# zrudnick/bramble

Hardware: AMD Instinct MI355X
Metric: projected alignments/sec vs GENCODE-scale annotation (higher is better)
Workload: dtype u32; 1 GPU; device-resident (inputs already in HBM, packed rows left in HBM): 10M paired-end 2x100 short reads (name-collated, unstranded) vs GENCODE-shaped synthetic annotation (250836 transcripts, 1684128 transcript-exon rows, 25 refs); BASELINE.json configs[1]; group_lanes=8, seed=0xb4a3b1e

## Files before the change

bramble_amd/csrc/abi.cpp:

```cpp
#include <hip/hip_runtime.h>

#include <algorithm>
#include <atomic>
#include <cstdio>
#include <cstdlib>
#include <cstring>
#include <functional>
#include <string>
#include <thread>
#include <unordered_map>
#include <vector>

#include "ctx.h"
#include "primary_pick.h"

int check_device(int device) {
  int n = 0;
  hipError_t e = hipGetDeviceCount(&n);
  if (e != hipSuccess || n <= 0 || device >= n) return BR_ERR_NO_DEVICE;
  return BR_OK;
}

template <typename T>
static int upload(void **dst, const std::vector<T> &src, size_t &acc) {
// ... 342 lines not shown
  return BR_OK;
}

extern "C" void br_ctx_free(br_ctx *c) {
  if (!c) return;
  (void)hipSetDevice(c->ix->device);
  for (auto &e : c->events) { (void)hipEventDestroy(e.a); (void)hipEventDestroy(e.b); }
  if (c->rb) (void)hipHostFree(c->rb);
  for (auto &S : c->stage) if (S.ready) (void)hipEventDestroy(S.ready);
  for (auto &S : c->in_slot) {
    if (S.ready) (void)hipEventDestroy(S.ready);
    if (S.rows_home) (void)hipEventDestroy(S.rows_home);
  }
  if (c->rows_busy) (void)hipEventDestroy(c->rows_busy);
  if (c->alt.busy) (void)hipEventDestroy(c->alt.busy);
  if (c->side2_stream) (void)hipStreamDestroy(c->side2_stream);
  if (c->side_stream) { (void)hipStreamDestroy(c->side_stream); for (auto &p : c->side_ev) for (auto &e : p) if (e) (void)hipEventDestroy(e); }
  if (c->run_stream) (void)hipStreamDestroy(c->run_stream);
  if (c->d2h_stream) (void)hipStreamDestroy(c->d2h_stream);
  if (c->copy_stream) (void)hipStreamDestroy(c->copy_stream);
  if (c->down_stream) (void)hipStreamDestroy(c->down_stream);
  for (int k = 0; k < 2; k++) if (c->ev_home[k]) (void)hipEventDestroy(c->ev_home[k]);
  delete c;
}

extern "C" int br_ctx_set_profiling(br_ctx *c, int enabled) {
  if (!c) return BR_ERR_INVALID_ARG;
  if (enabled && !c->profiling) for (int k = 0; k < BR_K_NUM; k++) { c->k_ms_sum[k] = 0; c->k_launches_sum[k] = 0; }
  c->profiling = enabled != 0;
  return BR_OK;
}
extern "C" int br_ctx_kernel_ms_sum(br_ctx *c, int which, double *ms, int64_t *launches) {
  if (!c || which < 0 || which >= BR_K_NUM) return BR_ERR_INVALID_ARG;
  if (ms) *ms = c->k_ms_sum[which];
  if (launches) *launches = c->k_launches_sum[which];
  return BR_OK;
}
extern "C" int br_ctx_set_param(br_ctx *c, const char *key, int64_t v) {
  if (!c || !key) return BR_ERR_INVALID_ARG;
  if (!strcmp(key, "group_lanes")) { if (v != 8 && v != 16 && v != 32 && v != 64) return BR_ERR_INVALID_ARG; c->group_lanes = (int)v; return BR_OK; }
  if (!strcmp(key, "direct_rows")) { c->direct_rows = v != 0; return BR_OK; }
  if (!strcmp(key, "small_batch")) { c->small_batch = v != 0; return BR_OK; }
  if (!strcmp(key, "speculate")) { c->speculate = v != 0; return BR_OK; }
  if (!strcmp(key, "speculate_n")) { if (v < 0) return BR_ERR_INVALID_ARG; c->speculate_n = v; return BR_OK; }
  if (!strcmp(key, "small_n")) { if (v < 0) return BR_ERR_INVALID_ARG; c->small_n = v; return BR_OK; }
  if (!strcmp(key, "deflate_dynamic")) { c->deflate_dynamic = v != 0; return BR_OK; }
  if (!strcmp(key, "bam_lanes")) { if (v != 0 && v != 4 && v != 8 && v != 16 && v != 32 && v != 64) return BR_ERR_INVALID_ARG; c->bam_lanes = (int)v; return BR_OK; }
  if (!strcmp(key, "ksw_fast")) { c->ksw_fast = v != 0; return BR_OK; }
  if (!strcmp(key, "ksw_tape_pct")) { if (v < 0 || v > 100) return BR_ERR_INVALID_ARG; c->ksw_tape_pct = (int)v; return BR_OK; }
  if (!strcmp(key, "ksw_tape_mb")) { if (v < 1) return BR_ERR_INVALID_ARG; c->ksw_tape_mb = v; return BR_OK; }
  if (!strcmp(key, "host_detail")) { c->host_detail = v != 0; return BR_OK; }
  if (!strcmp(key, "split_spoil")) { if (v < 0 || v > 1000000) return BR_ERR_INVALID_ARG; c->split_spoil = (int)v; return BR_OK; }
  if (!strcmp(key, "side_cap")) { if (v < 64) return BR_ERR_INVALID_ARG; c->d_side_cap = (uint64_t)v; return BR_OK; }
  if (!strcmp(key, "blocks_per_cu")) { if (v < 1 || v > 64) return BR_ERR_INVALID_ARG; c->blocks_per_cu = (int)v; return BR_OK; }
  return BR_ERR_INVALID_ARG;
}
extern "C" int br_ctx_kernel_ms(br_ctx *c, int which, double *ms, int32_t *launches) {
  if (!c || which < 0 || which >= BR_K_NUM) return BR_ERR_INVALID_ARG;
  if (ms) *ms = c->k_ms[which];
  if (launches) *launches = c->k_launches[which];
  return BR_OK;
}
extern "C" int br_ctx_ksw_diag(br_ctx *c, uint64_t out[16]) {
  if (!c || !out) return BR_ERR_INVALID_ARG;
  memcpy(out, c->ksw_diag, sizeof(c->ksw_diag));
  out[7] = (uint32_t)c->rb->ksw_left_after;
  return BR_OK;
}

extern "C" int br_ctx_rescue_stats(br_ctx *c, uint64_t out[4]) {
  if (!c || !out) return BR_ERR_INVALID_ARG;
  memcpy(out, c->rescue_stats, sizeof(c->rescue_stats));
  return BR_OK;
}
extern "C" int br_ctx_last_counters(br_ctx *c, uint64_t out[8]) {
  if (!c || !out) return BR_ERR_INVALID_ARG;
  memcpy(out, c->counters, sizeof(c->counters));
  return BR_OK;
}

extern "C" int br_pin_host(void *p, size_t bytes) {
  if (!p || !bytes) return BR_ERR_INVALID_ARG;
  HIPCHK(hipHostRegister(p, bytes, hipHostRegisterDefault));
  return BR_OK;
}
extern "C" int br_unpin_host(void *p) {
  if (!p) return BR_ERR_INVALID_ARG;
  HIPCHK(hipHostUnregister(p));
  return BR_OK;
}

extern "C" uint32_t br_primary_pick(const char *name, size_t len, uint32_t n_tied) {
  return n_tied ? br::primary_pick((const uint8_t *)name, len, n_tied) : 0;
}

extern "C" uint32_t br_row_mapq(uint32_t nh, int long_reads) {
  if (!long_reads) return nh == 1 ? 255u : nh == 2 ? 3u : (nh == 3 || nh == 4) ? 1u : 0u;
  return nh > 1 ? 0u : 3u;
}

extern "C" int br_device_warmup(int device) {
  int rc = check_device(device);
  if (rc) return rc;
  HIPCHK(hipSetDevice(device));
  HIPCHK(hipFree(nullptr));
  return BR_OK;
// ... 16 lines not shown
```

bramble_amd/csrc/ctx.h:

```cpp
#pragma once
#include <hip/hip_runtime.h>

#include <atomic>
#include <cassert>
#include <string>
#include <vector>

#include "../../include/bramble_amd.h"
#include "device_types.h"
#include "devmem.h"
#include "kernels.h"

using namespace br;

struct br_index {
  int device = -1;
  std::vector<std::string> names;
  std::vector<uint32_t> lengths;
  uint32_t n_refs = 0;
  bool has_seq = false;
  std::vector<uint32_t> slab_off, s_start, s_pmax, s_tid, tx_first, bin_off;
  std::vector<uint4> t_bin;
  std::vector<uint4> s_row, tx_ex;
  std::vector<uint8_t> seq_pool;
  void *d_slab_off = nullptr, *d_s_start = nullptr, *d_s_pmax = nullptr, *d_bin_off = nullptr, *d_t_bin = nullptr, *d_s_tid = nullptr,
       *d_s_row = nullptr, *d_tx_ex = nullptr, *d_tx_first = nullptr, *d_seq_pool = nullptr;
  size_t device_bytes = 0;
  DevIndex dev{};
};

struct KEvent { int which; hipEvent_t a, b; };

struct ReadBack {
  uint64_t scan[5];
  uint64_t counters[4];
  uint64_t small[TOT_SMALL_CNT + 4];
  uint64_t direct_cnt[GD_COUNTER_WORDS];
  uint64_t side[2];
  uint64_t wide_cigar;
  uint64_t rescue_n[2];
  uint64_t rescue_stats[2];
  uint32_t ksw_bins[16];
  uint64_t ksw_left_after;
  uint64_t parse_n[3];
  uint64_t parse_seq;
  uint64_t parse_max;
  uint64_t bam[2];
  uint64_t deflate_total;
  uint64_t host_groups, host_max, host_pool;
  uint64_t sam_bad, sam_bytes;
};

struct br_ctx {
  const br_index *ix = nullptr;
  int group_lanes = 8;
  int bam_lanes = 0;
  int blocks_per_cu = 8;
  int split_spoil = 0;
  int n_cu = 256;
  bool profiling = false;
  std::vector<KEvent> events; size_t events_used = 0;
  double k_ms[BR_K_NUM] = {0}; int32_t k_launches[BR_K_NUM] = {0};
  double k_ms_sum[BR_K_NUM] = {0}; int64_t k_launches_sum[BR_K_NUM] = {0};
  uint64_t counters[8] = {0};
  uint64_t rescue_stats[4] = {0};
  DevBuf seg, meta, head, head2, fast_flag, fast_pre, n_matches, ranges, mask, match_off, cig_base, tile_sums, totals, counters_d;
  DevBuf m_tid, m_aux, m_p, m_x, m_b, m_cigoff, cig_arena, big_list, n_big, m_aln;
  DevBuf bam_aux, bam_base, bam_len, bam_off, bam_out, bam_end;
  struct StageSlot { DevBuf blob, off, len; hipEvent_t ready = nullptr; std::vector<uint64_t> h_off; int64_t n = 0; };
  StageSlot stage[3];
  hipStream_t copy_stream = nullptr;
  struct InSlot {
    DevBuf ref_id, ref_start, flags, xs, ts, cigar_off64, cigar, mate_ref, mate_start, name_off64, names, lqseq, seq_off64, seqs;
    DevBuf cigar_off, name_off, seq_off, mate_idx, group_off, seq_src, isnew, group_pre;
    hipEvent_t ready = nullptr, rows_home = nullptr;
    int64_t n = -1; uint64_t n_words = 0, n_name = 0, n_seq = 0; bool has_seq = false, staged = false, rows_pending = false;
    PinnedVec<uint4> h_a; PinnedVec<uint64_t> h_c, h_row_off; PinnedVec<uint32_t> h_pool; PinnedVec<uint4> h_x;
    PinnedVec<int32_t> h_mate, h_clip; PinnedVec<double> h_sim;
  };
  InSlot in_slot[2];
  hipStream_t run_stream = nullptr, d2h_stream = nullptr;
  hipEvent_t rows_busy = nullptr;
  bool rows_busy_set = false;
  struct RowSetAlt { DevBuf pk_a, pk_x, pk_sim, pk_clip, pk_ch, pool, row_off; hipEvent_t busy = nullptr; bool busy_set = false; } alt;
  int host_detail = 0;
  DevBuf z_slots, z_sizes, z_off, z_dense, z_dense_alt, z_tabs, z_tokens;
  DevBuf inf_out, inf_blocks, inf_tabs, inf_cnt; bool inf_tabs_ready = false;
  DevBuf sp_entry, sp_entry2, sp_exit, sp_nmap, sp_nunm, sp_ended, sp_redo, sp_pre, sp_small, sp_off, sp_len;
  DevBuf sf_names, sf_name_off, sf_len, sf_long, sf_small, sf_tmp, sf_text[2];
  int32_t sf_n_names = 0;
  int sf_which = 0;
  int z_dense_which = 0;
  hipStream_t down_stream = nullptr; hipEvent_t ev_home[2] = {nullptr, nullptr}; std::atomic<bool> home_pending[2] = {{false}, {false}};
  int deflate_dynamic = 1;
  int64_t speculate_n = 4194304;
  int speculate = 1;
  int64_t hist_n = 0; uint64_t hist[4] = {0, 0, 0, 0}; bool hist_simf = false;
  int small_batch = 1;
  int64_t small_n = 65536;
  DevBuf walk_list, pmask, pbit, pick;
  int direct_rows = 1;
  DevBuf d_fm, d_nkept, d_desc, d_hi0, d_clspos, d_rnd, d_side, d_sidectr;
  uint64_t d_side_cap = 0;
  int d_side_attempts = 0;
  bool last_direct = false;
  bool want_x = false;
  ProjectArgs dA{}; DirectArgs dD{}; int64_t d_kept = 0, d_simple = 0;
  DevBuf r_rec, pk_a, pk_c, pk_x, pk_sim, pk_clip;
  DevBuf pool, pool_sizes, pool_off, pk_ch;
  bool last_aux_cols = false;
  bool wide_valid = false;
  bool detail_valid = false;
  const int32_t *last_l_qseq = nullptr;
  int32_t last_long_reads = 0;
  int64_t last_n_pool = 0;
  bool z_tabs_ready = false;
  DevBuf p_ncig, p_name_len, p_isnew, p_group_pre, p_small, p_big, p_seq_len, p_ref_map;
  uint8_t *h_bam[2] = {nullptr, nullptr}; size_t h_bam_cap[2] = {0, 0}; int h_bam_next = 0;
  BigPinned h_bam_mem[2];
  int64_t last_n_rows = 0, last_n_aln = 0;
  br_device_bam last_bam{};
  br_device_rows last_rows{}; const uint32_t *last_group_off = nullptr; int64_t last_n_groups = 0; hipStream_t last_stream = nullptr;
  DevBuf fa_stats, fa_n_prob, fa_seq_bytes, fa_prob_off, fa_seqarena_off, fa_probs, fa_results, fa_seq_arena, fa_clip_ops,
      fa_ideal_cap, fa_scratch, fa_srcs, fa_want, b_seq_off, b_seqs, b_seq_src;
  DevBuf ksw_desc, ksw_dp, ksw_left, ksw_cnt, ksw_group, ksw_tape, ksw_raw;
  int ksw_fast = 1;
  hipStream_t side_stream = nullptr, side2_stream = nullptr;
  static constexpr int SIDE_EV = 8;
  hipEvent_t side_ev[SIDE_EV][2] = {}; int side_live = 0;
  uint32_t ksw_groups[KSW_N_BINS] = {0};
  int64_t ksw_tape_mb = 49152;
  int ksw_tape_pct = 100;
  uint64_t ksw_diag[16] = {0};
  DevBuf n_rows, row_off, aln_group;
  DevBuf r_input, r_nh, r_hi, r_mapq, r_group, r_mate_tid, r_mate_pos,
      r_isize, r_tid, r_pos, r_ncig, r_strand, r_sim, r_clip, r_junc, r_refc, r_cigoff, cigar_out;
  DevBuf r_paired, r_same, r_first, r_primary;
  DevBuf b_name_off, b_names;
  DevBuf b_ref_id, b_ref_start, b_flags, b_xs, b_ts, b_cigar_off, b_cigar, b_mate_idx, b_group_off, b_lqseq;
  ReadBack *rb = nullptr;
  PinnedVec<int32_t> h_input, h_clip, h_junc, h_refc, h_mate_tid, h_mate_pos, h_isize;
  PinnedVec<uint32_t> h_tid, h_pos, h_nh, h_hi, h_mapq, h_group, h_cigar;
  PinnedVec<int8_t> h_strand;
  PinnedVec<uint64_t> h_cigoff;
  PinnedVec<double> h_sim;
  PinnedVec<uint8_t> h_primary, h_paired, h_same, h_first;
  std::vector<br_projected> h_proj;
  PinnedVec<uint8_t> g_host; DevBuf g_dev;
  PinnedVec<uint4> g_a, g_x; PinnedVec<uint2> g_c; PinnedVec<uint32_t> g_pool, g_cig; PinnedVec<double> g_sim;
  bool rows_to_host = false, rows_at_host = false;
};

struct Prof {
  br_ctx *c; hipStream_t st;
  hipStream_t cur = nullptr;
  int begin(int which, hipStream_t on = nullptr) {
// ... 70 lines not shown
```

bramble_amd/csrc/direct_kernels.inc:

```

#define WAVE_SYNC()                                                \
  do {                                                             \
    __builtin_amdgcn_fence(__ATOMIC_RELEASE, "workgroup");         \
    __builtin_amdgcn_wave_barrier();                               \
    __builtin_amdgcn_fence(__ATOMIC_ACQUIRE, "workgroup");         \
  } while (0)

__global__ void __launch_bounds__(256) k_name_seed(DirectArgs D) {
  const int64_t g = (int64_t)blockIdx.x * blockDim.x + threadIdx.x;
  if (g >= D.n_groups) return;
  const uint32_t a0 = D.group_off[g];
  const uint32_t no = D.name_off[a0];
  Mt64Lazy gen;
  gen.seed(hash_bytes(D.names + no, D.name_off[a0 + 1] - no));
  D.rnd0[g] = gen();
}
__device__ __forceinline__ uint32_t pick_from(uint64_t z0, const uint8_t *name, uint64_t len, uint32_t n) {
  uint64_t hi, lo;
  mul64wide(z0, (uint64_t)n, hi, lo);
  if (lo < (uint64_t)n) {
    const uint64_t thr = (0 - (uint64_t)n) % (uint64_t)n;
    if (lo < thr) return primary_pick(name, len, n);
  }
  return (uint32_t)hi;
// ... 479 lines not shown
    if (small) {
#pragma unroll
      for (int k = 0; k < 4; k++) {
        const uint32_t i = a0 + (uint32_t)k, r = r4[k];
        if (r) {
        const uint32_t pf = f4[k];
        const bool paired = (pf & PF_PAIRED) != 0;
        const uint32_t u = paired ? r / 2 : r;
        uint32_t prim = 0;
        if (have_prim && idx != 0xffffffffu) { if (idx < u) { prim = idx + 1u; idx = 0xffffffffu; } else idx -= u; }
        D.gd[i] = make_uint2(pf | (prim << 8), total);
        D.hi0[i] = run + 1u;
        if (paired) {
          const uint32_t m = (uint32_t)mi4[k], mk = m - a0;
          const uint32_t pfm = mk < na ? (mk == 0 ? f4[0] : mk == 1 ? f4[1] : mk == 2 ? f4[2] : f4[3]) : (uint32_t)D.pflag[m];
          D.gd[m] = make_uint2(pfm | (prim << 8), total);
          D.hi0[m] = run + 2u;
        }
        run += r;
        }
      }
    } else {
      for (uint32_t i = a0; i < a1; i++) {
        const uint32_t r = D.n_rows[i];
        if (!r) continue;
        const uint32_t pf = D.pflag[i];
        const bool paired = (pf & PF_PAIRED) != 0;
        const uint32_t u = paired ? r / 2 : r;
        uint32_t prim = 0;
        if (have_prim && idx != 0xffffffffu) { if (idx < u) { prim = idx + 1u; idx = 0xffffffffu; } else idx -= u; }
        D.gd[i] = make_uint2(pf | (prim << 8), total);
        D.hi0[i] = run + 1u;
        if (paired) {
          const uint32_t m = (uint32_t)D.mate_idx[i];
          D.gd[m] = make_uint2((uint32_t)D.pflag[m] | (prim << 8), total);
          D.hi0[m] = run + 2u;
        }
        run += r;
      }
    }
  }
  __shared__ unsigned long long sh_c[4][2];
  uniq = wave_sum(uniq); dropped = wave_sum(dropped);
  if ((threadIdx.x & 63) == 0) { sh_c[threadIdx.x >> 6][0] = uniq; sh_c[threadIdx.x >> 6][1] = dropped; }
  __syncthreads();
  if (threadIdx.x == 0) {
    const unsigned long long u = sh_c[0][0] + sh_c[1][0] + sh_c[2][0] + sh_c[3][0], dr = sh_c[0][1] + sh_c[1][1] + sh_c[2][1] + sh_c[3][1];
    uint64_t *slot = D.counters + GD_SLOT0 + (size_t)(blockIdx.x & (GD_SLOTS - 1)) * GD_SLOT_STRIDE;
    if (u) atomicAdd((unsigned long long *)&slot[0], u);
    if (dr) atomicAdd((unsigned long long *)&slot[1], dr);
  }
}

__global__ void __launch_bounds__(256) k_expand_rows(DirectArgs D) {
  __shared__ uint32_t sh_pre[4][64], sh_v[4][64];
  const int lane = threadIdx.x & 63, wv = threadIdx.x >> 6;
  const int64_t a = (int64_t)blockIdx.x * blockDim.x + threadIdx.x;
  if (D.m_aln_cap && D.tot[TOT_MATCHES] > D.m_aln_cap) return;
  if (D.side_used[1]) return;
  uint32_t nk = 0, pos = 0, v = 0;
  bool fast = false;
  if (a < D.n_aln) nk = D.n_kept[a];
  if (nk) {
    fast = D.fast_flag[a] >> 31;
    pos = D.cls_pos[a];
    const uint32_t y = D.pflag[a];
    const bool is_mate = (y & PF_MATE) != 0;
    const uint32_t leader = is_mate ? (uint32_t)D.mate_idx[a] : (uint32_t)a;
    D.dpos[a] = make_uint2((uint32_t)D.row_off[leader] + (is_mate ? 1u : 0u), pos);
    v = (y & PF_BIG) ? 0xffffffffu : (uint32_t)a;
  }
  sh_v[wv][lane] = v;
#pragma unroll
  for (int c = 0; c < 2; c++) {
    const uint32_t mine = (nk && fast == (c == 0)) ? nk : 0u;
    const uint64_t have = __ballot(mine != 0u);
    if (!have) continue;
    uint32_t inc = mine;
#pragma unroll
    for (int d = 1; d < 64; d <<= 1) { const uint32_t up = __shfl_up(inc, d); if (lane >= d) inc += up; }
    const uint32_t total = __shfl(inc, 63), first = __shfl(pos, (int)__builtin_ctzll(have));
    __builtin_amdgcn_wave_barrier();
    sh_pre[wv][lane] = inc - mine;
    WAVE_SYNC();
    for (uint32_t e = lane; e < total; e += 64) {
      int l = 0;
#pragma unroll
      for (int st = 32; st; st >>= 1) if (sh_pre[wv][l + st] <= e) l += st;
      D.m_aln[first + e] = sh_v[wv][l];
    }
  }
}

template <int CLS>
__global__ void __launch_bounds__(256, CLS == 1 ? 8 : 5) k_emit_rows(ProjectArgs A, DirectArgs D, int64_t first, int64_t n_end) {
  __shared__ uint32_t sh_cig[CLS == 1 ? 1 : 256 * LDS_SLOT];
  __shared__ uint16_t sh_mops[CLS == 1 ? 1 : 256];
  if (CLS != 1) {
    sh_mops[threadIdx.x] = (uint16_t)((merge_action(threadIdx.x >> 4, threadIdx.x & 15u) << 8) | merge_ops(threadIdx.x >> 4, threadIdx.x & 15u));
    __syncthreads();
  }
  const int64_t e64 = first + (int64_t)blockIdx.x * blockDim.x + threadIdx.x;
  if (e64 >= n_end) return;
  const DevIndex &ix = A.ix;
  const DevCfg &cfg = A.cfg;
  typedef uint32_t ntl4 __attribute__((ext_vector_type(4)));
  typedef uint32_t ntl2 __attribute__((ext_vector_type(2)));
  const uint32_t a = __builtin_nontemporal_load(D.m_aln + e64);
  if (a == 0xffffffffu) return;
  const ntl4 hd_ = __builtin_nontemporal_load((const ntl4 *)(A.head + a)), rg_ = __builtin_nontemporal_load((const ntl4 *)(A.ranges + a));
  const ntl2 f_ = __builtin_nontemporal_load((const ntl2 *)(D.fm + a)), gd_ = __builtin_nontemporal_load((const ntl2 *)(D.gd + a)), dp_ = __builtin_nontemporal_load((const ntl2 *)(D.dpos + a));
  const uint4 hd = make_uint4(hd_.x, hd_.y, hd_.z, hd_.w), rg = make_uint4(rg_.x, rg_.y, rg_.z, rg_.w);
  const uint2 f = make_uint2(f_.x, f_.y), gd = make_uint2(gd_.x, gd_.y), dp = make_uint2(dp_.x, dp_.y);
  const uint4 E = make_uint4(gd.x, gd.y, dp.x, dp.y);
  const uint32_t is_fast = CLS == 1;
  uint4 hd2 = make_uint4(0, 0, 0, 0);
  uint32_t c0 = 0, c1 = 0;
  RealCig rc;
  if (CLS != 1) { hd2 = A.head2[a]; c0 = A.cigar_off[a]; c1 = A.cigar_off[a + 1]; }
  else if (hd.z == 2) hd2 = A.head2[a];
  const uint32_t n_seg = hd.z, rid = hd.w >> 2;
  const uint2 q0 = make_uint2(hd.x, hd.y);
  const int st0 = (n_seg == 1) ? ST_ONLY : ST_FIRST;
  const uint32_t n0 = rg.y - rg.x;
  if (CLS != 1) rc.fetch(A.cigar + c0, c1 - c0);
  const uint32_t k = (uint32_t)e64 - E.w;
  const uint64_t fmask = (uint64_t)f.x | ((uint64_t)f.y << 32);
  const uint32_t item = kth_set_bit64(fmask, k);
  const int s = item < n0 ? 0 : 1;
  const uint32_t row = s == 0 ? rg.x + item : rg.z + (item - n0);
  const uint4 r_a = ix.s_row[2 * (size_t)row], r_b = ix.s_row[2 * (size_t)row + 1];
  const uint32_t gs = r_a.x, gend = r_a.y;
  const uint4 pay = make_uint4(r_b.x, r_b.y, r_a.w, r_b.z);
  uint32_t c = 0;
  {
    for (uint64_t m2 = fmask; m2;) {
      uint32_t t8[8]; bool ok[8];
#pragma unroll
      for (int u = 0; u < 8; u++) {
        ok[u] = m2 != 0;
        const uint32_t b = ok[u] ? (uint32_t)(__ffsll((long long)m2) - 1) : item;
        m2 &= m2 - 1;
        t8[u] = ix.s_tid[b < n0 ? rg.x + b : rg.z + (b - n0)];
      }
#pragma unroll
      for (int u = 0; u < 8; u++) c += (ok[u] && t8[u] < pay.x) ? 1u : 0u;
    }
  }
  Hit h0;
  classify(s == 1, st0, q0.x, q0.y, gs, gend, pay.z, cfg, h0);
  if (is_fast) {
    const uint32_t os = q0.x > gs ? q0.x : gs, oe = q0.y < gend ? q0.y : gend;
    uint32_t ml = oe - os, pos = h0.pos, r_ins = h0.right_ins, junc_in = 0;
    bool r_exact = h0.right_ins == 0 && h0.right_gap == 0;
    if (n_seg == 2) {
      const uint2 q1 = make_uint2(hd2.x, hd2.y);
      const uint4 e1 = next_row(make_uint4(gs, gend, pay.z, 0), make_uint2(r_a.z, r_b.w), s == 1);
      Hit hh;
      classify(s == 1, ST_LAST, q1.x, q1.y, e1.x, e1.y, e1.z, cfg, hh);
      ml += (q1.y < e1.y ? q1.y : e1.y) - q1.x;
      pos = s == 0 ? h0.pos : hh.pos;
      r_ins = hh.right_ins; r_exact = hh.right_ins == 0 && hh.right_gap == 0;
      junc_in = 2;
    }
    uint32_t w0, w1 = 0, w2 = 0, n_out;
    if (h0.left_ins) { w0 = CIG_GEN(h0.left_ins, OP_S); w1 = CIG_GEN(ml, OP_M); n_out = 2; if (r_ins) { w2 = CIG_GEN(r_ins, OP_S); n_out = 3; } }
    else { w0 = CIG_GEN(ml, OP_M); n_out = 1; if (r_ins) { w1 = CIG_GEN(r_ins, OP_S); n_out = 2; } }
    const uint32_t junc = junc_in + ((h0.left_ins == 0 && h0.left_gap == 0) ? 1u : 0u) + (r_exact ? 1u : 0u);
    uint64_t cref = (uint64_t)w0 | ((uint64_t)w1 << 32);
    if (n_out == 3) {
      cref = D.cig_base[a] + (uint64_t)c * (n_seg == 2 ? 3u + 2u * 10u : 1u + 2u * 6u);
      uint32_t *slot = A.cig_arena + cref;
      slot[0] = w0; slot[1] = w1; slot[2] = w2;
    }
    write_row(D, E, a, c, pay.x, pos, n_out, s == 1, cref, junc, ml);
    return;
  }
  if (CLS == 1) return;
  ReadCtx rd;
  rd.n_seg = n_seg; rd.seg = A.seg + (size_t)c0 + (size_t)a; rd.real = A.cigar + c0; rd.n_real = c1 - c0; rd.q12 = hd2;
  const uint4 *Ex = ix.tx_ex + pay.w;
  const uint32_t i0 = pay.y & 0x7fffffffu;
  CandOut p1;
  bool plain = false;
  const uint32_t sb = ix.slab_off[2 * rid + s], se = ix.slab_off[2 * rid + s + 1];
  if (n_seg == 1) { p1.alive = true; p1.fwpos = h0.pos; p1.rcpos = h0.pos; p1.n_seg = 1; p1.n_gex = 1; p1.i_lastm = i0; p1.last_right_ins = h0.right_ins; p1.last_right_gap = h0.right_gap; }
  else if (!cfg.long_reads && !cfg.ignore_small_exons) {
    plain = true;
    p1.alive = true; p1.fwpos = h0.pos; p1.rcpos = h0.pos; p1.n_seg = n_seg; p1.n_gex = n_seg; p1.i_lastm = i0;
    p1.last_right_ins = 0; p1.last_right_gap = 0;
  }
  else p1 = walk_pass1(ix, cfg, rd, Ex, s == 1, sb, se, i0, make_uint4(gs, gend, pay.z, 0), make_uint2(r_a.z, r_b.w), q0, h0);
  const uint32_t ideal_cap = 4u * n_seg + 2u;
  const uint32_t cap = rd.n_real + 2u * ideal_cap;
  const uint64_t slot_off = D.cig_base[a] + (uint64_t)c * cap;
  uint32_t *slot = A.cig_arena + slot_off;
  uint32_t *lds = &sh_cig[(CLS == 1 ? 0 : threadIdx.x) * LDS_SLOT];
  const bool ideal_lds = ideal_cap <= LDS_IDEAL;
  uint32_t *ideal = ideal_lds ? lds : slot + rd.n_real + ideal_cap;
  Acc acc; IdealSink sk;
  sk.init(ideal);
// ... 50 lines not shown
```

bramble_amd/csrc/kernels.h:

```cpp
#pragma once
#include <hip/hip_runtime.h>
#include <stdint.h>

#include "device_types.h"
#include "ksw_types.h"
#include "scan_kernels.h"

namespace br {

enum {
  TOT_MATCHES = 0,
  TOT_ARENA = 1,
  TOT_SIMPLE = 2,
  TOT_ROWS = 3,
  TOT_RAW = 4,
  TOT_RESCUE_PROB = 5,
  TOT_RESCUE_SEQ = 6,
  TOT_WIDE_CIGAR = 7,
  TOT_SMALL_CNT = 8,
  TOT_PARSE_CIGAR = 12,
  TOT_PARSE_NAMES = 13,
  TOT_PARSE_GROUPS = 14,
  TOT_PARSE_SEQ = 15,
  TOT_BAM_LONG = 16,
// ... 107 lines not shown
};

struct ScanArgs {
  int64_t n;
  const uint32_t *src32;
  const uint32_t *cigar_off;
  const uint32_t *ideal_cap;
  const uint32_t *fast_flag;
  uint64_t *tile_sums;
  int64_t n_tiles;
};

#define RM_NCIG 0x00ffffffu
#define RM_MINUS (1u << 24)
#define RM_PAIRED (1u << 25)
#define RM_SAME (1u << 26)
#define RM_FIRST (1u << 27)
#define RM_PRIMARY (1u << 28)
struct PairArgs {
  int64_t n_groups, n_aln, n_rows_total;
  int32_t long_reads;
  const uint32_t *group_off;
  const uint32_t *aln_group;
  const int32_t *mate_idx;
  const uint32_t *match_off;
  const uint32_t *n_matches;
  const uint32_t *m_tid;
  const uint2 *m_p, *m_x;
  const uint4 *m_b;
  const uint64_t *m_cigoff;
  uint32_t *n_rows;
  uint64_t *pick;
  uint8_t *pbit;
  uint64_t *pmask;
  const uint64_t *row_off;
  uint4 *r_rec;
  uint4 *r_a;
  uint2 *r_c;
  uint4 *r_x;
  double *r_sim;
  int32_t *r_clip;
  uint64_t *counters;
  const uint64_t *tot;
  uint64_t lim_m, lim_c;
  uint64_t lim_r;
};
__device__ __forceinline__ bool rows_over(const uint64_t *tot, uint64_t lim_r) { return tot && tot[TOT_ROWS] > lim_r; }
#define RR_HI 0x0fffffffu
#define RR_PRIMARY (1u << 28)
#define RR_PAIRED (1u << 29)
#define RR_SAME (1u << 30)
#define RR_FIRST (1u << 31)

enum : uint32_t { PF_PAIRED = 1, PF_SAME = 2, PF_MATE = 4, PF_BIG = 8 };
struct DirectArgs {
  int64_t n_aln, n_groups;
  const uint32_t *group_off;
  const uint32_t *aln_group;
  const int32_t *mate_idx;
  const uint32_t *n_matches;
  const uint64_t *mask;
  const uint4 *ranges;
  const uint32_t *fast_flag;
  const uint32_t *s_tid;
  const uint32_t *big_list; const uint32_t *n_big;
  uint2 *fm;
  uint32_t *n_kept;
  uint32_t *n_rows;
  uint8_t *pflag;
  uint2 *side;
  uint64_t side_cap;
  uint32_t *pm_list, *pm_n;
  unsigned long long *side_used;
  uint32_t *cls_pos;
  uint64_t *cig_base;
  uint64_t *row_off;
  const uint32_t *name_off; const uint8_t *names;
  uint64_t *rnd0;
  uint2 *gd;
  uint2 *dpos;
  uint32_t *hi0;
  uint64_t *counters;
  const uint64_t *tot;
  uint32_t *m_aln;
  uint64_t m_aln_cap;
  uint4 *r_a; uint2 *r_c;
  uint4 *r_x;
};
#define GD_SLOTS 16
#define GD_SLOT0 16
#define GD_SLOT_STRIDE 16
#define GD_COUNTER_WORDS (GD_SLOT0 + GD_SLOTS * GD_SLOT_STRIDE)
void launch_name_seed(hipStream_t st, const DirectArgs &D);
void launch_pair_mask(hipStream_t st, const DirectArgs &D, int wide_blocks);
void launch_big_collect(hipStream_t st, const ProjectArgs &A, const DirectArgs &D, int n_blocks);
void launch_pair_big(hipStream_t st, const DirectArgs &D, int n_blocks);
void launch_scan5(hipStream_t st, const DirectArgs &D, uint64_t *tile_sums, uint64_t *total_out5);
void launch_group_desc(hipStream_t st, const DirectArgs &D);
void launch_expand_rows(hipStream_t st, const DirectArgs &D);
void launch_emit_rows(hipStream_t st, const ProjectArgs &A, const DirectArgs &D, int64_t n_kept, int64_t n_simple, int part);
void launch_big_emit(hipStream_t st, const ProjectArgs &A, const DirectArgs &D, int n_blocks);

struct PoolArgs {
  int64_t n_rows;
  const uint4 *r_a; const uint2 *r_c;
  const uint32_t *arena;
  uint32_t *sizes;
  const uint64_t *off;
  uint2 *c_out;
  uint32_t *pool;
};

struct WideArgs {
  int64_t n_rows, n_aln;
  int32_t long_reads;
  const uint4 *r_a; const uint2 *r_c; const uint4 *r_x;
  const double *r_sim; const int32_t *r_clip;
  const uint32_t *pool;
  const uint32_t *aln_group;
  const int32_t *l_qseq;
  int32_t *w_input;
  uint32_t *w_nh, *w_hi, *w_mapq, *w_group;
  int32_t *w_mate_tid, *w_mate_pos, *w_isize;
  uint32_t *w_tid, *w_pos, *w_ncig;
  int8_t *w_strand;
  double *w_sim;
  int32_t *w_clip, *w_junc, *w_refc;
  uint8_t *w_paired, *w_same, *w_first, *w_primary;
  const uint64_t *w_cigoff;
  uint32_t *w_cigar;
};

struct StatsArgs {
  DevIndex ix;
  int64_t n_aln;
  const int32_t *ref_id;
  const uint32_t *cigar_off;
  const uint2 *seg;
// ... 166 lines not shown
```

bramble_amd/csrc/pipeline.cpp:

```cpp
#include <algorithm>
#include <cstring>
#include <vector>

#include "ctx.h"

int ensure_side_stream(br_ctx *c) {
  if (c->side_stream) return BR_OK;
  HIPCHK(hipStreamCreateWithPriority(&c->side_stream, hipStreamNonBlocking, 0));
  for (auto &p : c->side_ev) for (auto &e : p) HIPCHK(hipEventCreateWithFlags(&e, hipEventDisableTiming));
  return BR_OK;
}

int run_ksw(br_ctx *c, hipStream_t st, const KswRun &R) {
  if (R.n_prob <= 0) return BR_OK;
  const uint64_t n_all = (uint64_t)R.n_prob;
  const uint64_t qmax = std::max<uint64_t>(R.qmax, 1), tmax = std::max<uint64_t>(R.tmax, 1);
  KswArgs K{};
  K.n_prob = R.n_prob; K.probs = R.probs; K.results = R.results; K.seq_arena = R.seq_arena; K.clip_ops = R.clip_ops;
  K.stats = R.stats;
  K.raw_out = R.raw_out; K.raw_n = R.raw_n; K.max_out = R.max_out; K.raw_cap = R.raw_cap;
  auto general = [&](uint64_t n_work, uint64_t q_hi, uint64_t t_hi, const uint32_t *list, const uint32_t *n_list) -> int {
    q_hi = std::max<uint64_t>(q_hi, 1); t_hi = std::max<uint64_t>(t_hi, 1);
    K.tmax = (uint32_t)t_hi;
    K.pmat_bytes = (size_t)(((q_hi + t_hi) * t_hi + 15) & ~15ull);
// ... 358 lines not shown
  RC(row_tail(c, st, b, P, pf, aux_cols, big, true, c->rows_to_host ? cap_m : 0));
  ReadBack *rb = c->rb;
  HIPCHK(hipMemcpyAsync(rb->small, d_tot, sizeof(rb->small), hipMemcpyDeviceToHost, st));
  HIPCHK(hipStreamSynchronize(st));
  for (int k = 0; k < 4; k++) { rb->scan[k] = rb->small[k]; rb->counters[k] = rb->small[TOT_SMALL_CNT + k]; }
  const uint64_t n_matches = rb->scan[TOT_MATCHES], n_cig_arena = rb->scan[TOT_ARENA], n_simple = rb->scan[TOT_SIMPLE], n_rows = rb->scan[TOT_ROWS];
  if (n_matches > cap_m || n_cig_arena > cap_c || n_rows > P.lim_r) return BR_RETRY_ORDINARY;
  if (big && (!dc.filter_by_similarity ? (n_simple > cover_s || n_matches - n_simple > cover_g) : n_matches > cover_m)) return BR_RETRY_ORDINARY;
  c->hist_simf = dc.filter_by_similarity != 0;
  c->hist_n = n; c->hist[0] = n_matches; c->hist[1] = n_cig_arena; c->hist[2] = n_simple; c->hist[3] = n_rows;
  if (!keep_events) RC(pf.collect());
  if (rb->counters[3]) return BR_ERR_UNSUPPORTED;
  finish_call(c, dc, b, out, n_matches, n_rows, n_cig_arena, aux_cols, &P);
  return BR_OK;
}

static int run_device_direct(br_ctx *c, const DevCfg &dc, const br_device_batch *b, hipStream_t st, br_device_rows *out, Prof &pf,
                             bool keep_events) {
  const br_index *ix = c->ix;
  const int64_t n = b->n_aln, ng = b->n_groups;
  const int64_t tiles = std::max<int64_t>(scan_tiles_for(std::max<int64_t>(n, ng) + 1), 1);
  RC(ensure_count_tables(c, b));
  RC(c->n_matches.ensure((size_t)n * 4 + 16));
  RC(c->tile_sums.ensure((size_t)tiles * 8 * 5));
  RC(c->counters_d.ensure((GD_COUNTER_WORDS + 4) * 8));
  uint64_t *const dz = c->counters_d.as<uint64_t>();
  uint32_t *const dz_nbig = (uint32_t *)(dz + GD_COUNTER_WORDS + 2);
  RC(c->walk_list.ensure((size_t)n * 4));
  RC(c->aln_group.ensure((size_t)n * 4)); RC(c->n_rows.ensure((size_t)n * 4 + 16)); RC(c->pbit.ensure((size_t)n + 16));
  RC(c->d_fm.ensure((size_t)n * sizeof(uint2) + (size_t)(n / 62 + 2) * 4));
  RC(c->d_nkept.ensure((size_t)n * 4)); RC(c->d_desc.ensure((size_t)n * sizeof(uint4)));
  RC(c->d_hi0.ensure((size_t)n * 4)); RC(c->d_clspos.ensure((size_t)n * 4)); RC(c->d_rnd.ensure((size_t)std::max<int64_t>(ng, 1) * 8));
  if (c->d_side_cap == 0) c->d_side_cap = std::max<uint64_t>((uint64_t)n / 4, 1u << 20);
  RC(c->d_side.ensure((size_t)c->d_side_cap * sizeof(uint2)));
  if (c->rows_busy_set && c->row_off.cap < (size_t)(n + 1) * 8) HIPCHK(hipEventSynchronize(c->rows_busy));
  RC(c->row_off.ensure((size_t)(n + 1) * 8));
  RC(ensure_side_stream(c));
  if (!c->side2_stream) HIPCHK(hipStreamCreateWithPriority(&c->side2_stream, hipStreamNonBlocking, 0));
  hipStream_t ax = c->side_stream, ax2 = c->side2_stream;
  uint64_t *d_tot = c->totals.as<uint64_t>();
  ReadBack *rb = c->rb;

  ProjectArgs A = count_args(c, dc, b);
  A.n_big = dz_nbig; A.walk_list = c->walk_list.as<uint32_t>(); A.n_walk = dz_nbig + 1;
  const bool have_names = b->names && b->name_off;
  DirectArgs D{};
  D.n_aln = n; D.n_groups = ng; D.group_off = b->group_off; D.aln_group = c->aln_group.as<uint32_t>(); D.mate_idx = b->mate_idx;
  D.n_matches = c->n_matches.as<uint32_t>(); D.mask = c->mask.as<uint64_t>(); D.ranges = c->ranges.as<uint4>();
  D.fast_flag = c->fast_flag.as<uint32_t>(); D.s_tid = ix->dev.s_tid; D.big_list = A.big_list; D.n_big = A.n_big;
  D.fm = c->d_fm.as<uint2>(); D.pm_list = (uint32_t *)(c->d_fm.as<uint2>() + n); D.pm_n = dz_nbig + 2; D.n_kept = c->d_nkept.as<uint32_t>(); D.n_rows = c->n_rows.as<uint32_t>(); D.pflag = c->pbit.as<uint8_t>();
  D.side = c->d_side.as<uint2>(); D.side_cap = c->d_side_cap; D.side_used = (unsigned long long *)(dz + GD_COUNTER_WORDS);
  D.cls_pos = c->d_clspos.as<uint32_t>(); D.cig_base = c->cig_base.as<uint64_t>(); D.row_off = c->row_off.as<uint64_t>();
  D.name_off = have_names ? b->name_off : nullptr; D.names = have_names ? b->names : nullptr; D.rnd0 = c->d_rnd.as<uint64_t>();
  D.gd = c->d_desc.as<uint2>(); D.dpos = c->d_desc.as<uint2>() + n; D.hi0 = c->d_hi0.as<uint32_t>(); D.counters = c->counters_d.as<uint64_t>(); D.tot = d_tot;

  SideWork seeds(c, st, ax2), pair_big(c, st, ax), group_desc(c, st, ax), big_emit(c, st, ax);
  HIPCHK(hipMemsetAsync(dz, 0, (GD_COUNTER_WORDS + 4) * 8, st));
  RC(pair_big.fork());
  RC(segment_stage(c, st, dc, b, pf));
  RC(pf.begin(BR_K_GROUP_IDS));
  launch_group_ids(st, ng, b->group_off, c->aln_group.as<uint32_t>());
  RC(pf.end());
  RC(count_pass(c, st, A, pf, true, true));
  if (c->rows_busy_set) { HIPCHK(hipStreamWaitEvent(st, c->rows_busy, 0)); }
  const int big_blocks = c->n_cu * 4;
  uint64_t kept = 0, arena = 0, n_simple = 0, n_rows = 0, n_raw = 0;
  bool expanded_ahead = false;
  if (have_names) {
    RC(seeds.fork());
    RC(pf.begin(BR_K_NAME_SEED, ax2));
    launch_name_seed(ax2, D);
    RC(pf.end());
    RC(seeds.done());
  }
  for (int attempt = 0;; attempt++) {
    if (attempt) {
      HIPCHK(hipMemsetAsync(dz, 0, (GD_COUNTER_WORDS + 2) * 8, st));
      HIPCHK(hipMemsetAsync(D.pm_n, 0, 4, st));
    }
    RC(pair_big.fork());
    RC(pf.begin(BR_K_PAIR_BIG, ax));
    launch_big_collect(ax, A, D, big_blocks);
    launch_pair_big(ax, D, big_blocks);
    RC(pf.end());
    RC(pair_big.done());
    RC(pf.begin(BR_K_PAIR_MASK));
    launch_pair_mask(st, D, c->n_cu * 2);
    RC(pf.end());
    RC(pair_big.join());
    RC(group_desc.fork());
    if (have_names) RC(seeds.join_on(ax));
    RC(pf.begin(BR_K_GROUP_DESC, ax));
    launch_group_desc(ax, D);
    RC(pf.end());
    RC(group_desc.done());
    RC(pf.begin(BR_K_SCAN));
    launch_scan5(st, D, c->tile_sums.as<uint64_t>(), d_tot);
    RC(pf.end());
    expanded_ahead = false;
    if (c->m_aln.cap >= 4) {
      D.m_aln = c->m_aln.as<uint32_t>(); D.m_aln_cap = c->m_aln.cap / 4;
      RC(pf.begin(BR_K_EXPAND_ROWS));
      launch_expand_rows(st, D);
      RC(pf.end());
      expanded_ahead = true;
    }
    HIPCHK(hipMemcpyAsync(rb->scan, d_tot, sizeof(rb->scan), hipMemcpyDeviceToHost, st));
    HIPCHK(hipMemcpyAsync(rb->side, dz + GD_COUNTER_WORDS, sizeof(rb->side), hipMemcpyDeviceToHost, st));
    HIPCHK(hipStreamSynchronize(st));
    c->d_side_attempts = attempt + 1;
    if (rb->side[1]) {
      if (attempt >= 3) return BR_ERR_CAPACITY;
      RC(group_desc.wait_host());
      c->d_side_cap = rb->side[0] + rb->side[0] / 4 + 4096;
      RC(c->d_side.ensure((size_t)c->d_side_cap * sizeof(uint2)));
      D.side = c->d_side.as<uint2>(); D.side_cap = c->d_side_cap;
      continue;
    }
    kept = rb->scan[TOT_MATCHES]; arena = rb->scan[TOT_ARENA]; n_simple = rb->scan[TOT_SIMPLE]; n_rows = rb->scan[TOT_ROWS]; n_raw = rb->scan[TOT_RAW];
    break;
  }
  if (n_raw >= 0xffffffffull || kept >= 0xffffffffull) return BR_ERR_CAPACITY;
  if (kept != n_rows) return BR_ERR_HIP;

  const size_t nr = (size_t)std::max<uint64_t>(n_rows, 1);
  if (c->rows_busy_set && (c->pk_a.cap < nr * sizeof(uint4) || c->pk_c.cap < nr * sizeof(uint2))) HIPCHK(hipEventSynchronize(c->rows_busy));
  RC(c->pk_a.ensure(nr * sizeof(uint4))); RC(c->pk_c.ensure(nr * sizeof(uint2)));
  if (expanded_ahead && kept > D.m_aln_cap) expanded_ahead = false;
  RC(c->m_aln.ensure(nr * 4)); RC(c->cig_arena.ensure((size_t)std::max<uint64_t>(arena, 1) * 4));
  const bool with_x = c->want_x;
  if (with_x) {
    if (c->rows_busy_set && c->pk_x.cap < nr * sizeof(uint4)) HIPCHK(hipEventSynchronize(c->rows_busy));
    RC(c->pk_x.ensure(nr * sizeof(uint4)));
  }
  A.cig_arena = c->cig_arena.as<uint32_t>();
  D.m_aln = c->m_aln.as<uint32_t>(); D.r_a = c->pk_a.as<uint4>(); D.r_c = c->pk_c.as<uint2>(); D.r_x = with_x ? c->pk_x.as<uint4>() : nullptr;
  D.m_aln_cap = 0;
  if (kept) {
    if (!expanded_ahead) {
      RC(pf.begin(BR_K_EXPAND_ROWS));
      launch_expand_rows(st, D);
      RC(pf.end());
    }
    RC(group_desc.join());
    RC(big_emit.fork());
    RC(pf.begin(BR_K_BIG_EMIT, ax));
    launch_big_emit(ax, A, D, big_blocks);
    RC(pf.end());
    RC(big_emit.done());
    RC(pf.begin(BR_K_EMIT_ROWS_SIMPLE));
    launch_emit_rows(st, A, D, (int64_t)kept, (int64_t)n_simple, 1);
    RC(pf.end());
    RC(pf.begin(BR_K_EMIT_ROWS));
    launch_emit_rows(st, A, D, (int64_t)kept, (int64_t)n_simple, 2);
    RC(pf.end());
    RC(big_emit.join());
  } else {
    RC(group_desc.join());
  }
  HIPCHK(hipMemcpyAsync(rb->direct_cnt, c->counters_d.p, sizeof(rb->direct_cnt), hipMemcpyDeviceToHost, st));
  HIPCHK(hipStreamSynchronize(st));
  if (!keep_events) RC(pf.collect());
  for (int k = 0; k < 4; k++) rb->counters[k] = rb->direct_cnt[k];
  for (int k = 0; k < GD_SLOTS; k++) { rb->counters[1] += rb->direct_cnt[GD_SLOT0 + k * GD_SLOT_STRIDE]; rb->counters[2] += rb->direct_cnt[GD_SLOT0 + k * GD_SLOT_STRIDE + 1]; }
  if (rb->counters[3]) return BR_ERR_UNSUPPORTED;
  c->hist_n = 0;
  finish_call(c, dc, b, out, n_raw, n_rows, arena, false);
  out->a = (const br_row_a *)c->pk_a.p; out->cigar = (const uint64_t *)c->pk_c.p; out->x = with_x ? (const br_row_x *)c->pk_x.p : nullptr;
  out->similarity_score = nullptr; out->clip_score = nullptr;
  c->detail_valid = with_x;
  c->last_direct = true; c->dA = A; c->dD = D; c->d_kept = (int64_t)kept; c->d_simple = (int64_t)n_simple;
  return BR_OK;
}

static int run_match_table(br_ctx *c, const DevCfg &dc, const br_device_batch *b, hipStream_t st, br_device_rows *out, Prof &pf,
                           bool keep_events) {
  const bool fa_mode = dc.use_fasta && dc.long_reads;
  const int64_t n = b->n_aln, ng = b->n_groups;
  const int64_t tiles = std::max<int64_t>(scan_tiles_for(std::max<int64_t>(n, ng) + 1), 1);
  RC(ensure_count_tables(c, b));
  RC(c->n_matches.ensure((size_t)n * 4)); RC(c->fast_pre.ensure((size_t)(n + 1) * 4)); RC(c->match_off.ensure((size_t)(n + 1) * 4));
  RC(c->tile_sums.ensure((size_t)tiles * 8 * 3)); RC(c->counters_d.ensure(4 * 8));
  RC(c->n_big.ensure(16)); RC(c->walk_list.ensure((size_t)n * 4));
  uint64_t *d_tot = c->totals.as<uint64_t>();
  ReadBack *rb = c->rb;

  RC(segment_stage(c, st, dc, b, pf));
  ProjectArgs A = count_args(c, dc, b);
  A.fast_pre = c->fast_pre.as<uint32_t>(); A.match_off = c->match_off.as<uint32_t>(); A.cig_base = c->cig_base.as<uint64_t>();
// ... 312 lines not shown
```

Before: 3.202 billion alignments/s.

## Precompute per-row item and transcript rank in expand_rows via shared-memory runs

Moves the per-row kth-set-bit selection and the transcript-id rank count out of the emit kernel and into k_expand_rows. There, each wave stages the transcript ids of the rows it expands in LDS and counts the smaller ids within each alignment's run using vectorized shared loads. The result is written as a compact 16-bit selector (item plus rank) into a new m_sel buffer. Emit no longer loads the fm mask and re-gathers s_tid for every set bit, which was quadratic per alignment. In exchange it adds an extra 2-byte-per-row buffer, a larger per-block LDS footprint, a chunked loop in expand, and a new rank_cap parameter.

```diff
diff --git a/bramble_amd/csrc/abi.cpp b/bramble_amd/csrc/abi.cpp
--- a/bramble_amd/csrc/abi.cpp
+++ b/bramble_amd/csrc/abi.cpp
@@ -418,6 +418,7 @@
   if (!strcmp(key, "host_detail")) { c->host_detail = v != 0; return BR_OK; }
   if (!strcmp(key, "split_spoil")) { if (v < 0 || v > 1000000) return BR_ERR_INVALID_ARG; c->split_spoil = (int)v; return BR_OK; }
   if (!strcmp(key, "side_cap")) { if (v < 64) return BR_ERR_INVALID_ARG; c->d_side_cap = (uint64_t)v; return BR_OK; }
+  if (!strcmp(key, "rank_cap")) { if (v < 64 || v > XR_CAP) return BR_ERR_INVALID_ARG; c->d_rank_cap = (uint32_t)v; return BR_OK; }
   if (!strcmp(key, "blocks_per_cu")) { if (v < 1 || v > 64) return BR_ERR_INVALID_ARG; c->blocks_per_cu = (int)v; return BR_OK; }
   return BR_ERR_INVALID_ARG;
 }
diff --git a/bramble_amd/csrc/ctx.h b/bramble_amd/csrc/ctx.h
--- a/bramble_amd/csrc/ctx.h
+++ b/bramble_amd/csrc/ctx.h
@@ -65,7 +65,7 @@
   uint64_t counters[8] = {0};
   uint64_t rescue_stats[4] = {0};
   DevBuf seg, meta, head, head2, fast_flag, fast_pre, n_matches, ranges, mask, match_off, cig_base, tile_sums, totals, counters_d;
-  DevBuf m_tid, m_aux, m_p, m_x, m_b, m_cigoff, cig_arena, big_list, n_big, m_aln;
+  DevBuf m_tid, m_aux, m_p, m_x, m_b, m_cigoff, cig_arena, big_list, n_big, m_aln, m_sel;
   DevBuf bam_aux, bam_base, bam_len, bam_off, bam_out, bam_end;
   struct StageSlot { DevBuf blob, off, len; hipEvent_t ready = nullptr; std::vector<uint64_t> h_off; int64_t n = 0; };
   StageSlot stage[3];
@@ -102,6 +102,7 @@
   int direct_rows = 1;
   DevBuf d_fm, d_nkept, d_desc, d_hi0, d_clspos, d_rnd, d_side, d_sidectr;
   uint64_t d_side_cap = 0;
+  uint32_t d_rank_cap = XR_CAP;
   int d_side_attempts = 0;
   bool last_direct = false;
   bool want_x = false;
diff --git a/bramble_amd/csrc/direct_kernels.inc b/bramble_amd/csrc/direct_kernels.inc
--- a/bramble_amd/csrc/direct_kernels.inc
+++ b/bramble_amd/csrc/direct_kernels.inc
@@ -555,14 +555,22 @@
   }
 }
 
+struct XrSh {
+  uint32_t tid[XR_CAP] __attribute__((aligned(16)));
+  uint2 fm[64];
+  uint32_t pre[64], pre_r[64], lo0[64], lo1[64], n0[64];
+  uint16_t so[64];
+};
 __global__ void __launch_bounds__(256) k_expand_rows(DirectArgs D) {
-  __shared__ uint32_t sh_pre[4][64], sh_v[4][64];
+  __shared__ XrSh sh_all[4];
   const int lane = threadIdx.x & 63, wv = threadIdx.x >> 6;
+  XrSh &S = sh_all[wv];
   const int64_t a = (int64_t)blockIdx.x * blockDim.x + threadIdx.x;
   if (D.m_aln_cap && D.tot[TOT_MATCHES] > D.m_aln_cap) return;
   if (D.side_used[1]) return;
-  uint32_t nk = 0, pos = 0, v = 0;
-  bool fast = false;
+  uint32_t nk = 0, pos = 0;
+  bool fast = false, is_big = false;
+  uint2 f = make_uint2(0, 0); uint4 rg = make_uint4(0, 0, 0, 0);
   if (a < D.n_aln) nk = D.n_kept[a];
   if (nk) {
     fast = D.fast_flag[a] >> 31;
@@ -571,26 +579,98 @@
     const bool is_mate = (y & PF_MATE) != 0;
     const uint32_t leader = is_mate ? (uint32_t)D.mate_idx[a] : (uint32_t)a;
     D.dpos[a] = make_uint2((uint32_t)D.row_off[leader] + (is_mate ? 1u : 0u), pos);
-    v = (y & PF_BIG) ? 0xffffffffu : (uint32_t)a;
-  }
-  sh_v[wv][lane] = v;
-#pragma unroll
+    is_big = (y & PF_BIG) != 0;
+    if (!is_big) { f = D.fm[a]; rg = D.ranges[a]; }
+  }
+  S.fm[lane] = f; S.lo0[lane] = rg.x; S.lo1[lane] = rg.z; S.n0[lane] = rg.y - rg.x;
+  const uint32_t a0 = (uint32_t)(a - lane);
+  const uint32_t cap = D.rank_cap < 64u ? 64u : D.rank_cap > (uint32_t)XR_CAP ? (uint32_t)XR_CAP : D.rank_cap;
+#pragma unroll 1
   for (int c = 0; c < 2; c++) {
     const uint32_t mine = (nk && fast == (c == 0)) ? nk : 0u;
     const uint64_t have = __ballot(mine != 0u);
     if (!have) continue;
-    uint32_t inc = mine;
-#pragma unroll
-    for (int d = 1; d < 64; d <<= 1) { const uint32_t up = __shfl_up(inc, d); if (lane >= d) inc += up; }
-    const uint32_t total = __shfl(inc, 63), first = __shfl(pos, (int)__builtin_ctzll(have));
+    const uint64_t bigs = __ballot(mine != 0u && is_big);
+    const uint32_t mine_r = is_big ? 0u : (mine > 64u ? 64u : mine), slots = (mine_r + 3u) & ~3u;
+    uint32_t inc = mine, inc_s = slots;
+#pragma unroll
+    for (int d = 1; d < 64; d <<= 1) { const uint32_t up = __shfl_up(inc, d), us = __shfl_up(inc_s, d); if (lane >= d) { inc += up; inc_s += us; } }
+    uint32_t inc_r = inc;
+    if (bigs) {
+      inc_r = mine_r;
+#pragma unroll
+      for (int d = 1; d < 64; d <<= 1) { const uint32_t up = __shfl_up(inc_r, d); if (lane >= d) inc_r += up; }
+    }
+    const uint32_t total = __shfl(inc, 63), total_r = __shfl(inc_r, 63), first = __shfl(pos, (int)__builtin_ctzll(have));
+    const uint32_t ex_r = inc_r - mine_r, ex_s = inc_s - slots;
     __builtin_amdgcn_wave_barrier();
-    sh_pre[wv][lane] = inc - mine;
+    S.pre[lane] = inc - mine; S.pre_r[lane] = ex_r; S.so[lane] = (uint16_t)ex_s;
     WAVE_SYNC();
-    for (uint32_t e = lane; e < total; e += 64) {
-      int l = 0;
-#pragma unroll
-      for (int st = 32; st; st >>= 1) if (sh_pre[wv][l + st] <= e) l += st;
-      D.m_aln[first + e] = sh_v[wv][l];
+    if (bigs) {
+      for (uint32_t e = lane; e < total; e += 64) {
+        int l = 0;
+#pragma unroll
+        for (int st = 32; st; st >>= 1) if (S.pre[l + st] <= e) l += st;
+        D.m_aln[first + e] = ((bigs >> l) & 1ull) ? 0xffffffffu : a0 + (uint32_t)l;
+      }
+    }
+    for (int l0 = 0; l0 < 64 && total_r != 0u;) {
+      const uint32_t base_e = __shfl(ex_r, l0), base_s = __shfl(ex_s, l0);
+      const bool fits = lane >= l0 && inc_r - base_e <= 64u * XR_ROUNDS && inc_s - base_s <= cap;
+      int l1 = l0 + (int)__popcll(__ballot(fits));
+      if (l1 == l0) l1 = l0 + 1;
+      const uint32_t end_e = l1 < 64 ? __shfl(ex_r, l1 & 63) : total_r;
+      l0 = l1;
+      if (end_e == base_e) continue;
+      uint32_t t[XR_ROUNDS], eo[XR_ROUNDS], pk[XR_ROUNDS];
+#pragma unroll
+      for (int r = 0; r < XR_ROUNDS; r++) {
+        eo[r] = 0xffffffffu; t[r] = 0; pk[r] = 0;
+        if (base_e + 64u * r >= end_e) continue;
+        const uint32_t j = base_e + 64u * r + (uint32_t)lane;
+        if (j < end_e) {
+          int l = 0;
+#pragma unroll
+          for (int st = 32; st; st >>= 1) if (S.pre_r[l + st] <= j) l += st;
+          const uint32_t k = j - S.pre_r[l];
+          const uint2 fl = S.fm[l];
+          const uint64_t fmask = (uint64_t)fl.x | ((uint64_t)fl.y << 32);
+          const uint32_t n_l = (uint32_t)__popcll(fmask);
+          const uint32_t item = kth_set_bit64(fmask, k < n_l ? k : 0u);
+          t[r] = D.s_tid[row_of_bit(item, S.lo0[l], S.lo1[l], S.n0[l])];
+          const uint32_t rs = (uint32_t)S.so[l] - base_s;
+          pk[r] = item | ((rs + k) << 6) | (rs << 16) | ((((n_l + 3u) >> 2) - 1u) << 26) | (k + 1u == n_l ? 1u << 30 : 0u);
+          eo[r] = first + S.pre[l] + k;
+          D.m_aln[eo[r]] = a0 + (uint32_t)l;
+        }
+      }
+#pragma unroll
+      for (int r = 0; r < XR_ROUNDS; r++) {
+        if (base_e + 64u * r >= end_e) continue;
+        if (eo[r] != 0xffffffffu) {
+          const uint32_t slot = (pk[r] >> 6) & 1023u, run_end = ((pk[r] >> 16) & 1023u) + 4u * (((pk[r] >> 26) & 15u) + 1u);
+          if (run_end <= (uint32_t)XR_CAP) {
+            S.tid[slot] = t[r];
+            if (pk[r] >> 30) for (uint32_t q = slot + 1u; q < run_end; q++) S.tid[q] = 0xffffffffu;
+          }
+        }
+      }
+      WAVE_SYNC();
+#pragma unroll
+      for (int r = 0; r < XR_ROUNDS; r++) {
+        if (base_e + 64u * r >= end_e) continue;
+        if (eo[r] != 0xffffffffu) {
+          const uint32_t rs = (pk[r] >> 16) & 1023u, run_end = rs + 4u * (((pk[r] >> 26) & 15u) + 1u);
+          uint32_t rank = 0;
+          if (run_end <= (uint32_t)XR_CAP)
+            for (uint32_t x = rs; x < run_end; x += 4) {
+              const uint4 v = *(const uint4 *)&S.tid[x];
+              rank += (v.x < t[r] ? 1u : 0u) + (v.y < t[r] ? 1u : 0u) + (v.z < t[r] ? 1u : 0u) + (v.w < t[r] ? 1u : 0u);
+            }
+          D.m_sel[eo[r]] = (uint16_t)((pk[r] & 63u) | (rank << 8));
+        }
+      }
+      WAVE_SYNC();
     }
   }
 }
@@ -610,12 +690,14 @@
   typedef uint32_t ntl4 __attribute__((ext_vector_type(4)));
   typedef uint32_t ntl2 __attribute__((ext_vector_type(2)));
   const uint32_t a = __builtin_nontemporal_load(D.m_aln + e64);
+  const uint32_t sel = __builtin_nontemporal_load(D.m_sel + e64);
   if (a == 0xffffffffu) return;
   const ntl4 hd_ = __builtin_nontemporal_load((const ntl4 *)(A.head + a)), rg_ = __builtin_nontemporal_load((const ntl4 *)(A.ranges + a));
-  const ntl2 f_ = __builtin_nontemporal_load((const ntl2 *)(D.fm + a)), gd_ = __builtin_nontemporal_load((const ntl2 *)(D.gd + a)), dp_ = __builtin_nontemporal_load((const ntl2 *)(D.dpos + a));
+  const ntl2 gd_ = __builtin_nontemporal_load((const ntl2 *)(D.gd + a));
+  const uint32_t rec0 = __builtin_nontemporal_load(&D.dpos[a].x);
   const uint4 hd = make_uint4(hd_.x, hd_.y, hd_.z, hd_.w), rg = make_uint4(rg_.x, rg_.y, rg_.z, rg_.w);
-  const uint2 f = make_uint2(f_.x, f_.y), gd = make_uint2(gd_.x, gd_.y), dp = make_uint2(dp_.x, dp_.y);
-  const uint4 E = make_uint4(gd.x, gd.y, dp.x, dp.y);
+  const uint2 gd = make_uint2(gd_.x, gd_.y);
+  const uint4 E = make_uint4(gd.x, gd.y, rec0, 0);
   const uint32_t is_fast = CLS == 1;
   uint4 hd2 = make_uint4(0, 0, 0, 0);
   uint32_t c0 = 0, c1 = 0;
@@ -627,29 +709,12 @@
   const int st0 = (n_seg == 1) ? ST_ONLY : ST_FIRST;
   const uint32_t n0 = rg.y - rg.x;
   if (CLS != 1) rc.fetch(A.cigar + c0, c1 - c0);
-  const uint32_t k = (uint32_t)e64 - E.w;
-  const uint64_t fmask = (uint64_t)f.x | ((uint64_t)f.y << 32);
-  const uint32_t item = kth_set_bit64(fmask, k);
+  const uint32_t item = sel & 0xffu, c = sel >> 8;
   const int s = item < n0 ? 0 : 1;
   const uint32_t row = s == 0 ? rg.x + item : rg.z + (item - n0);
   const uint4 r_a = ix.s_row[2 * (size_t)row], r_b = ix.s_row[2 * (size_t)row + 1];
   const uint32_t gs = r_a.x, gend = r_a.y;
   const uint4 pay = make_uint4(r_b.x, r_b.y, r_a.w, r_b.z);
-  uint32_t c = 0;
-  {
-    for (uint64_t m2 = fmask; m2;) {
-      uint32_t t8[8]; bool ok[8];
-#pragma unroll
-      for (int u = 0; u < 8; u++) {
-        ok[u] = m2 != 0;
-        const uint32_t b = ok[u] ? (uint32_t)(__ffsll((long long)m2) - 1) : item;
-        m2 &= m2 - 1;
-        t8[u] = ix.s_tid[b < n0 ? rg.x + b : rg.z + (b - n0)];
-      }
-#pragma unroll
-      for (int u = 0; u < 8; u++) c += (ok[u] && t8[u] < pay.x) ? 1u : 0u;
-    }
-  }
   Hit h0;
   classify(s == 1, st0, q0.x, q0.y, gs, gend, pay.z, cfg, h0);
   if (is_fast) {
diff --git a/bramble_amd/csrc/kernels.h b/bramble_amd/csrc/kernels.h
--- a/bramble_amd/csrc/kernels.h
+++ b/bramble_amd/csrc/kernels.h
@@ -183,6 +183,8 @@
 #define RR_SAME (1u << 30)
 #define RR_FIRST (1u << 31)
 
+#define XR_CAP 768
+#define XR_ROUNDS 8
 enum : uint32_t { PF_PAIRED = 1, PF_SAME = 2, PF_MATE = 4, PF_BIG = 8 };
 struct DirectArgs {
   int64_t n_aln, n_groups;
@@ -214,7 +216,9 @@
   uint64_t *counters;
   const uint64_t *tot;
   uint32_t *m_aln;
+  uint16_t *m_sel;
   uint64_t m_aln_cap;
+  uint32_t rank_cap;
   uint4 *r_a; uint2 *r_c;
   uint4 *r_x;
 };
diff --git a/bramble_amd/csrc/pipeline.cpp b/bramble_amd/csrc/pipeline.cpp
--- a/bramble_amd/csrc/pipeline.cpp
+++ b/bramble_amd/csrc/pipeline.cpp
@@ -434,6 +434,7 @@
   D.side = c->d_side.as<uint2>(); D.side_cap = c->d_side_cap; D.side_used = (unsigned long long *)(dz + GD_COUNTER_WORDS);
   D.cls_pos = c->d_clspos.as<uint32_t>(); D.cig_base = c->cig_base.as<uint64_t>(); D.row_off = c->row_off.as<uint64_t>();
   D.name_off = have_names ? b->name_off : nullptr; D.names = have_names ? b->names : nullptr; D.rnd0 = c->d_rnd.as<uint64_t>();
+  D.rank_cap = c->d_rank_cap;
   D.gd = c->d_desc.as<uint2>(); D.dpos = c->d_desc.as<uint2>() + n; D.hi0 = c->d_hi0.as<uint32_t>(); D.counters = c->counters_d.as<uint64_t>(); D.tot = d_tot;
 
   SideWork seeds(c, st, ax2), pair_big(c, st, ax), group_desc(c, st, ax), big_emit(c, st, ax);
@@ -480,8 +481,8 @@
     launch_scan5(st, D, c->tile_sums.as<uint64_t>(), d_tot);
     RC(pf.end());
     expanded_ahead = false;
-    if (c->m_aln.cap >= 4) {
-      D.m_aln = c->m_aln.as<uint32_t>(); D.m_aln_cap = c->m_aln.cap / 4;
+    if (c->m_aln.cap >= 4 && c->m_sel.cap >= 2) {
+      D.m_aln = c->m_aln.as<uint32_t>(); D.m_sel = c->m_sel.as<uint16_t>(); D.m_aln_cap = std::min(c->m_aln.cap / 4, c->m_sel.cap / 2);
       RC(pf.begin(BR_K_EXPAND_ROWS));
       launch_expand_rows(st, D);
       RC(pf.end());
@@ -509,14 +510,14 @@
   if (c->rows_busy_set && (c->pk_a.cap < nr * sizeof(uint4) || c->pk_c.cap < nr * sizeof(uint2))) HIPCHK(hipEventSynchronize(c->rows_busy));
   RC(c->pk_a.ensure(nr * sizeof(uint4))); RC(c->pk_c.ensure(nr * sizeof(uint2)));
   if (expanded_ahead && kept > D.m_aln_cap) expanded_ahead = false;
-  RC(c->m_aln.ensure(nr * 4)); RC(c->cig_arena.ensure((size_t)std::max<uint64_t>(arena, 1) * 4));
+  RC(c->m_aln.ensure(nr * 4)); RC(c->m_sel.ensure(nr * 2)); RC(c->cig_arena.ensure((size_t)std::max<uint64_t>(arena, 1) * 4));
   const bool with_x = c->want_x;
   if (with_x) {
     if (c->rows_busy_set && c->pk_x.cap < nr * sizeof(uint4)) HIPCHK(hipEventSynchronize(c->rows_busy));
     RC(c->pk_x.ensure(nr * sizeof(uint4)));
   }
   A.cig_arena = c->cig_arena.as<uint32_t>();
-  D.m_aln = c->m_aln.as<uint32_t>(); D.r_a = c->pk_a.as<uint4>(); D.r_c = c->pk_c.as<uint2>(); D.r_x = with_x ? c->pk_x.as<uint4>() : nullptr;
+  D.m_aln = c->m_aln.as<uint32_t>(); D.m_sel = c->m_sel.as<uint16_t>(); D.r_a = c->pk_a.as<uint4>(); D.r_c = c->pk_c.as<uint2>(); D.r_x = with_x ? c->pk_x.as<uint4>() : nullptr;
   D.m_aln_cap = 0;
   if (kept) {
     if (!expanded_ahead) {
```

Measured after the change: 3.119 billion alignments/s. 2.6% lower.
